# cloudflare/sliceslice-rs

Hardware: AMD Instinct MI355X
Metric: haystack GB/s scanned (and % HBM roofline), 16-byte needle, 1/2/4/8 MI355X (higher is better)
Workload: dtype u8

## Files before the change

sliceslice-rs_amd/csrc/batched_kernels.hpp:

```cpp
#pragma once
#include "batched_types.hpp"

namespace ss {

constexpr uint32_t kPlanSliceMajorMax = 8;

constexpr uint32_t kPlanSampleTiles = 1024, kPlanSampleBytes = 4096, kPlanSampleBlocks = 64;
__device__ __forceinline__ uint8_t class_from_count(uint32_t cnt, uint32_t total)
{
    if (cnt == 0) return 0;
    const uint32_t ratio = total / cnt;
    const uint32_t bits = 31u - (uint32_t)__builtin_clz(ratio);
    return (uint8_t)(15u - (bits < 15u ? bits : 15u));
}
struct BatchClasses {
    uint32_t hist[256];
    uint32_t done, pad[15];
    uint8_t cls[256];
};
__global__ void __launch_bounds__(kBlock) batch_sample_kernel(const uint8_t *haystacks, const uint64_t *hay_begin, const uint64_t *hay_end,
                                                               uint64_t count, BatchClasses *out, unsigned long long *h_tag,
                                                               unsigned long long tag)
{
    __shared__ uint32_t h[kWavesPerBlock][256];
    __shared__ uint32_t s_total;
    __shared__ int s_last;
    for (int k = threadIdx.x; k < kWavesPerBlock * 256; k += kBlock) (&h[0][0])[k] = 0;
    if (threadIdx.x == 0) s_total = 0;
    __syncthreads();
    const int lane = threadIdx.x & (kWave - 1), wave = threadIdx.x / kWave;
    constexpr uint32_t kPerWave = kPlanSampleTiles / (kPlanSampleBlocks * kWavesPerBlock);
    for (uint32_t t = 0; t < kPerWave; ++t) {
        const uint64_t j = ((uint64_t)blockIdx.x * kWavesPerBlock + wave) * kPerWave + t;
        if (count < kPlanSampleTiles && j >= count * ((kPlanSampleTiles + count - 1) / count)) break;
        const uint64_t prob = count >= kPlanSampleTiles ? j * count / kPlanSampleTiles : j % count;
        const uint64_t h0 = hay_begin[prob], h1 = hay_end[prob];
        if (h1 <= h0) continue;
        const uint64_t len = h1 - h0;
        uint64_t off = 0, take = len;
        if (len > kPlanSampleBytes) {
            const uint64_t frac = ((uint32_t)j * 2654435761u) >> 8;
            off = (uint64_t)(((unsigned __int128)(len - kPlanSampleBytes) * frac) >> 24);
            take = kPlanSampleBytes;
        } else if (count < kPlanSampleTiles && j >= count) {
            continue;
        }
        const uint8_t *p = haystacks + h0 + off + (uint64_t)lane * 64;
        const uint64_t mine = (uint64_t)lane * 64 < take ? take - (uint64_t)lane * 64 : 0;
        if (mine >= 64) {
#pragma unroll
            for (int q = 0; q < 16; ++q) {
                const uint32_t w = reinterpret_cast<const UnalignedU32 *>(p + 4 * q)->v;
                atomicAdd(&h[wave][w & 0xFF], 1u);
                atomicAdd(&h[wave][(w >> 8) & 0xFF], 1u);
                atomicAdd(&h[wave][(w >> 16) & 0xFF], 1u);
                atomicAdd(&h[wave][w >> 24], 1u);
            }
        } else {
            for (uint64_t q = 0; q < mine; ++q) atomicAdd(&h[wave][p[q]], 1u);
        }
    }
    __syncthreads();
    const uint32_t part = h[0][threadIdx.x] + h[1][threadIdx.x] + h[2][threadIdx.x] + h[3][threadIdx.x];
    if (part) __hip_atomic_fetch_add(&out->hist[threadIdx.x], part, __ATOMIC_RELAXED, __HIP_MEMORY_SCOPE_AGENT);
    __threadfence();
    __syncthreads();
    if (threadIdx.x == 0)
        s_last = __hip_atomic_fetch_add(&out->done, 1u, __ATOMIC_ACQ_REL, __HIP_MEMORY_SCOPE_AGENT) + 1u == kPlanSampleBlocks;
    __syncthreads();
    if (!s_last) return;
    __threadfence();
    const uint32_t mine = __hip_atomic_exchange(&out->hist[threadIdx.x], 0u, __ATOMIC_RELAXED, __HIP_MEMORY_SCOPE_AGENT);
    uint32_t sum = mine;
#pragma unroll
    for (int o = 32; o > 0; o >>= 1) sum += __shfl_xor(sum, o);
    if (lane == 0) atomicAdd(&s_total, sum);
    __syncthreads();
    out->cls[threadIdx.x] = class_from_count(mine, s_total);
    __threadfence_system();
    __syncthreads();
    if (threadIdx.x == 0) {
        __hip_atomic_store(&out->done, 0u, __ATOMIC_RELAXED, __HIP_MEMORY_SCOPE_AGENT);
        if (h_tag) __hip_atomic_store(h_tag, tag, __ATOMIC_RELEASE, __HIP_MEMORY_SCOPE_SYSTEM);
    }
}

__global__ void __launch_bounds__(kBlock) batch_plan_kernel(const BatchArgs a, uint64_t count, BatchDesc *descs,
                                                             uint32_t nslices, uint32_t min_tiles, int tile_pieces, PlanStats *stats,
                                                             const uint8_t *cls, BatchCold *colds)
{
    __shared__ uint8_t s_class[256];
    __shared__ uint32_t s_max, s_maxt;
    __shared__ unsigned long long s_sum;
    if (threadIdx.x == 0) {
        s_max = s_maxt = 0;
        s_sum = 0;
    }
    if (cls) {
        s_class[threadIdx.x] = cls[threadIdx.x];
    } else {
        constexpr ClassPlanes P = make_class_planes();
        const uint32_t t = threadIdx.x, w = t >> 5;
        uint32_t lo = P.lo[0], hi = P.hi[0];
#pragma unroll
        for (uint32_t k = 1; k < 8; ++k) {
            lo = w == k ? P.lo[k] : lo;
            hi = w == k ? P.hi[k] : hi;
        }
        s_class[t] = (uint8_t)(((lo >> (t & 31)) & 1u) | (((hi >> (t & 31)) & 1u) << 1));
    }
    const uint64_t prob = (uint64_t)blockIdx.x * kBlock + threadIdx.x;
    const bool live = prob < count;
    const uint64_t pi = live ? prob : 0;
    const uint64_t h0 = a.hay_begin[pi], h1 = a.hay_end[pi];
    const uint64_t n0 = a.needle_begin[pi], n1 = a.needle_end[pi];
    const uint64_t given = a.position ? a.position[pi] : 0;
    __syncthreads();
    uint64_t tiles = 0;
    const bool free_pair = cls != nullptr && a.position == nullptr;
    if (stats) {
        uint32_t eff = 0;
        if (live) eff = plan_one(a, pi, h0, h1, n0, n1, given, descs, nslices, min_tiles, tile_pieces, s_class, &tiles, free_pair, colds);
        if (eff != 0) {
            atomicMax(&s_max, eff);
            atomicMax(&s_maxt, tiles > 0xffffffffull ? 0xffffffffu : (uint32_t)tiles);
            atomicAdd(&s_sum, (unsigned long long)tiles);
        }
        __syncthreads();
        if (threadIdx.x == 0 && s_max != 0) {
            atomicMax(&stats->max_slices, s_max);
            atomicMax(&stats->max_tiles, s_maxt);
            atomicAdd(reinterpret_cast<unsigned long long *>(&stats->total_tiles), s_sum);
        }
        return;
    }
    if (live) (void)plan_one(a, pi, h0, h1, n0, n1, given, descs, nslices, min_tiles, tile_pieces, s_class, &tiles, free_pair, colds);
}

__global__ void __launch_bounds__(kBlock) batch_cold_kernel(const BatchArgs a, const BatchDesc *__restrict__ descs, uint64_t count,
                                                             BatchCold *colds, const uint8_t *cls, int find)
{
    __shared__ uint8_t s_class[256];
    if (cls) {
        s_class[threadIdx.x] = cls[threadIdx.x];
    } else {
        s_class[threadIdx.x] = (uint8_t)rarity_class4((uint8_t)threadIdx.x);
    }
    __syncthreads();
    const uint64_t prob = (uint64_t)blockIdx.x * kBlock + threadIdx.x;
    if (prob >= count) return;
    const BatchDesc d = descs[prob];
    BatchCold c;
    c.order_idx[0] = c.order_idx[1] = c.order_val[0] = c.order_val[1] = 0;
    c.tail16[0] = c.tail16[1] = c.tail16[2] = c.tail16[3] = 0;
    c.norder = c.exact_len = 0;
    c.pad[0] = c.pad[1] = find ? ~0u : 0u;
    if ((d.per >> 32) != 0 && ((d.bytes >> 24) & 1) == 0) {
        const uint8_t *needle = a.needles + d.needle_off + d.anchor;
        const uint64_t nrel = d.n - d.anchor;
        const uint32_t lim = nrel < (uint64_t)kRefineWindow ? (uint32_t)nrel : (uint32_t)kRefineWindow;
        const uint32_t pos2 = 4 * ((d.shifts >> 6) & 3) + ((d.shifts >> 4) & 3), pos3 = 4 * ((d.shifts >> 10) & 3) + ((d.shifts >> 8) & 3);
        uint32_t b[kRefineWindow], k[kRefineWindow];
#pragma unroll
        for (int K = 0; K < kRefineWindow; ++K) b[K] = needle[(uint32_t)K < lim ? K : 0];
#pragma unroll
        for (int K = 0; K < kRefineWindow; ++K) k[K] = s_class[b[K]];
        uint32_t valid = 0;
#pragma unroll
        for (int K = 1; K < kRefineWindow; ++K)
            if ((uint32_t)K < lim && (uint32_t)K != pos2 && (uint32_t)K != pos3) valid |= 1u << K;
        uint64_t i0 = 0, i1 = 0, v0 = 0, v1 = 0;
        uint32_t m = 0, used = 0, far_used = 0;
        auto emit = [&](uint32_t K, uint32_t byte) {
            const uint32_t sh = 8 * (m & 7);
            if (m < 8) { i0 |= (uint64_t)K << sh; v0 |= (uint64_t)byte << sh; }
            else { i1 |= (uint64_t)K << sh; v1 |= (uint64_t)byte << sh; }
            ++m;
            used |= 1u << K;
        };
#pragma unroll 1
        for (uint32_t cl = 0; cl < 16; ++cl) {
#pragma unroll
            for (int K = 16; K < kRefineWindow; ++K)
                if (((valid >> K) & 1u) && k[K] == cl && far_used < kFarFirst) { emit(K, b[K]); ++far_used; }
        }
#pragma unroll 1
        for (uint32_t cl = 0; cl < 16; ++cl) {
#pragma unroll
            for (int K = 1; K < 16; ++K)
                if (((valid >> K) & 1u) && k[K] == cl && m < 15) emit(K, b[K]);
        }
#pragma unroll 1
        for (uint32_t cl = 0; cl < 16; ++cl) {
#pragma unroll
            for (int K = 16; K < kRefineWindow; ++K)
                if (((valid >> K) & 1u) && !((used >> K) & 1u) && k[K] == cl && m < 15) emit(K, b[K]);
        }
        c.norder = m;
        c.order_idx[0] = i0; c.order_idx[1] = i1;
        c.order_val[0] = v0; c.order_val[1] = v1;
        if (nrel <= 16) {
            const uint32_t behind = (uint32_t)nrel;
            const uint32_t back = (uint32_t)(d.anchor < 16 - behind ? d.anchor : 16 - behind);
            const uint32_t el = behind + back;
            c.exact_len = el | (back << 8);
            uint32_t t[16];
#pragma unroll
            for (uint32_t j = 0; j < 16; ++j) t[j] = (needle - back)[j < el ? j : 0];
#pragma unroll
            for (uint32_t j = 0; j < 16; ++j) t[j] = j < el ? t[j] : 0u;
#pragma unroll
            for (int j = 0; j < 4; ++j) c.tail16[j] = t[4 * j] | (t[4 * j + 1] << 8) | (t[4 * j + 2] << 16) | (t[4 * j + 3] << 24);
        }
    }
    colds[prob] = c;
}

struct __attribute__((aligned(64))) PlanCtl {
    unsigned long long run_word;
    uint32_t tally[2];
    uint32_t pad[12];
};
static_assert(sizeof(PlanCtl) == 64, "a line of its own");
struct __attribute__((aligned(128))) PlanState {
    struct __attribute__((aligned(64))) Half {
        uint64_t word;
        uint64_t pad[7];
    } half[2];
};
static_assert(sizeof(PlanState) == 128, "a problem's state: a cache line of its own, one half per run parity");
extern "C" __device__ unsigned long long ss_llvm_dispatch_id(void) __asm("llvm.amdgcn.dispatch.id");
__device__ __forceinline__ unsigned long long plan_run_identity()
{
    const uint64_t queue = (uint64_t)(uintptr_t)__builtin_amdgcn_queue_ptr() >> 12;
    return ((queue & 0x7FFFFFFull) << 36) | (ss_llvm_dispatch_id() & ((1ull << 36) - 1ull));
}

#ifndef SS_BATCH_WAVES_MAX
#define SS_BATCH_WAVES_MAX 4
#endif
template <int U, bool FIND = false, bool PLAN = false, bool MULTI = PLAN>
__global__ void __attribute__((amdgpu_waves_per_eu(4, SS_BATCH_WAVES_MAX))) __launch_bounds__(kBlock)
scan_batched_plan_kernel(const BatchArgs a, const BatchDesc *__restrict__ descs, uint32_t count, uint32_t nslices, BatchCold *colds,
                         PlanCtl *ctl, PlanState *states, unsigned long long *h_tally, uint32_t run)
{
    constexpr bool COUNTED = PLAN;
    __shared__ __attribute__((aligned(16))) uint8_t s_needle[kWavesPerBlock * kNeedleLds];
    __shared__ unsigned long long s_wg[kWavesPerBlock];
    const uint32_t w = blockIdx.x;
    const bool slice_major = nslices <= kPlanSliceMajorMax;
    uint32_t prob, slice;
    if (slice_major) {
        slice = w / count;
        prob = w - slice * count;
    } else {
        prob = w / nslices;
        slice = w - prob * nslices;
    }
    BatchCold *rec = colds + prob;
    const BatchDesc *dp = descs + prob;
    const bool peek = !FIND && slice_major && slice != 0;
    int seen0 = 0, seen1 = 0;
    if (MULTI) {
        if (peek) {
            seen0 = __hip_atomic_load(reinterpret_cast<int *>(&states[prob].half[0].word), __ATOMIC_RELAXED, __HIP_MEMORY_SCOPE_AGENT);
            seen1 = __hip_atomic_load(reinterpret_cast<int *>(&states[prob].half[1].word), __ATOMIC_RELAXED, __HIP_MEMORY_SCOPE_AGENT);
        }
    } else if (peek) {
        seen0 = __hip_atomic_load(reinterpret_cast<int *>(&rec->pad[1]), __ATOMIC_RELAXED, __HIP_MEMORY_SCOPE_AGENT);
    }
    BatchDesc d = *dp;
    unsigned long long run_word = 0;
    static_assert(PLAN || !MULTI, "only plans have runs");
    constexpr bool multi = MULTI;
    if (multi) __asm__ volatile("s_load_dwordx2 %0, %1, 0x0\n\ts_waitcnt lgkmcnt(0)" : "=s"(run_word) : "s"(ctl) : "memory");
    if (COUNTED) {
        pin_hot_fields(d);
        if ((threadIdx.x & (kWave - 1)) == 0)
            __hip_atomic_store(&s_wg[threadIdx.x / kWave], FIND ? ~0ull : 0ull, __ATOMIC_RELAXED, __HIP_MEMORY_SCOPE_WORKGROUP);
    }
    uint32_t parity = 0;
    if (multi) {
        const unsigned long long me = plan_run_identity();
        const bool mine = (run_word >> 1) == me;
        parity = mine ? (uint32_t)(run_word & 1ull) : (uint32_t)(run_word & 1ull) ^ 1u;
        if (blockIdx.x == 0 && threadIdx.x == 0 && !mine) {
            if (h_tally) {
                const uint32_t total = __hip_atomic_exchange(&ctl->tally[parity ^ 1u], 0u, __ATOMIC_RELAXED, __HIP_MEMORY_SCOPE_AGENT);
                __hip_atomic_store(h_tally, ((unsigned long long)run << 32) | total, __ATOMIC_RELAXED, __HIP_MEMORY_SCOPE_SYSTEM);
            }
            __hip_atomic_store(&ctl->run_word, (me << 1) | parity, __ATOMIC_RELAXED, __HIP_MEMORY_SCOPE_AGENT);
        }
    }
    const uint32_t eff = (uint32_t)(d.per >> 32), per = (uint32_t)d.per;
    const bool shared = MULTI && eff > 1;
    const int seen = MULTI ? (parity ? seen1 : seen0) : seen0;
    int *found = FIND ? nullptr : (shared ? reinterpret_cast<int *>(&states[prob].half[parity].word) : reinterpret_cast<int *>(&rec->pad[1]));
    void *sink = FIND ? (shared ? static_cast<void *>(&states[prob].half[parity].word) : static_cast<void *>(&rec->pad[0])) : static_cast<void *>(found);
    const uint32_t mis = d.shifts & 15;
    const uint64_t npieces = ((mis + d.end + 15) / 16 + 63) / 64;
    const uint64_t ntiles = (npieces + kWavesPerBlock * U - 1) / (kWavesPerBlock * U);
    if (slice >= eff) {
        if (COUNTED && eff == 0 && slice == 0 && threadIdx.x == 0) {
            if (FIND) a.best[prob] = d.n == 0 ? 0ull : ~0ull;
            else a.found[prob] = (int)d.shifts;
        }
        return;
    }
    uint64_t t0, te, step;
    bool work = true;
    if (slice_major) {
        t0 = (uint64_t)slice * per;
        te = t0 + per < ntiles ? t0 + per : ntiles;
        step = 1;
        work = __builtin_amdgcn_readfirstlane(seen) == 0;
    } else {
        t0 = slice;
        te = ntiles;
        step = eff;
    }
    work = work && t0 < te;
    if (!work) return;
    const bool opener = MULTI && eff > 1 && slice == 0 && threadIdx.x == 0;
    if (opener) {
        __hip_atomic_store(&states[prob].half[parity ^ 1u].word, FIND ? ~0ull : 0ull, __ATOMIC_RELAXED, __HIP_MEMORY_SCOPE_AGENT);
        if (FIND) (void)__hip_atomic_exchange(a.best + prob, ~0ull, __ATOMIC_RELAXED, __HIP_MEMORY_SCOPE_AGENT);
        else (void)__hip_atomic_exchange(a.found + prob, 0, __ATOMIC_RELAXED, __HIP_MEMORY_SCOPE_AGENT);
    }

    if (work) {
        Problem pr;
        hot_problem(d, mis, npieces, pr);
        constexpr bool READY = PLAN;
        typename std::conditional<READY, ColdInPlanT<MULTI>, ColdInCall>::type cold;
        if constexpr (READY)
            cold = ColdInPlanT<MULTI>{dp, colds + prob, a.needles, MULTI && eff > 1 ? (FIND ? static_cast<void *>(a.best + prob) : static_cast<void *>(a.found + prob)) : nullptr,
                              MULTI && eff > 1 && h_tally ? &ctl->tally[parity] : nullptr};
        else cold = ColdInCall{dp, colds + prob, a.needles, FIND ? static_cast<void *>(a.best + prob) : static_cast<void *>(a.found + prob)};
        void *wg_sink = COUNTED && eff == 1 ? static_cast<void *>(&s_wg[threadIdx.x / kWave]) : nullptr;
        if ((d.bytes >> 24) & 1) scan_tiles<0, 0, true, U, 1, FIND, false, true>(pr, cold, s_needle, t0, step, te, sink, wg_sink);
        else scan_tiles<kQDynamic, 0, false, U, 1, FIND, false, true>(pr, cold, s_needle, t0, step, te, sink, wg_sink);
    }
    if (opener) {
        __asm__ volatile("s_waitcnt vmcnt(0)" ::: "memory");
        if (FIND) {
            const uint64_t v = __hip_atomic_load(&states[prob].half[parity].word, __ATOMIC_RELAXED, __HIP_MEMORY_SCOPE_AGENT);
            if (v != ~0ull) __hip_atomic_fetch_min(a.best + prob, v, __ATOMIC_RELAXED, __HIP_MEMORY_SCOPE_AGENT);
        } else {
            const int v = __hip_atomic_load(reinterpret_cast<int *>(&states[prob].half[parity].word), __ATOMIC_RELAXED, __HIP_MEMORY_SCOPE_AGENT);
            if (v != 0) (void)__hip_atomic_exchange(a.found + prob, 1, __ATOMIC_RELAXED, __HIP_MEMORY_SCOPE_AGENT);
        }
    }
    if (COUNTED && eff == 1) {
        __syncthreads();
        if (threadIdx.x == 0) {
            unsigned long long mine = FIND ? ~0ull : 0ull;
#pragma unroll
            for (int k = 0; k < kWavesPerBlock; ++k) {
                const unsigned long long v = __hip_atomic_load(&s_wg[k], __ATOMIC_RELAXED, __HIP_MEMORY_SCOPE_WORKGROUP);
                mine = FIND ? (v < mine ? v : mine) : (mine | v);
            }
            if (FIND) a.best[prob] = mine;
            else a.found[prob] = mine != 0;
            if (MULTI) {
                __hip_atomic_store(&states[prob].half[0].word, FIND ? ~0ull : 0ull, __ATOMIC_RELAXED, __HIP_MEMORY_SCOPE_AGENT);
                __hip_atomic_store(&states[prob].half[1].word, FIND ? ~0ull : 0ull, __ATOMIC_RELAXED, __HIP_MEMORY_SCOPE_AGENT);
            }
        }
    }
}

__global__ void __launch_bounds__(kBlock) scan_pairs_kernel(const BatchArgs a, uint64_t count)
{
    const uint64_t prob = (uint64_t)blockIdx.x * kBlock + threadIdx.x;
    if (prob >= count) return;
    const uint64_t h0 = a.hay_begin[prob], n0 = a.needle_begin[prob];
    const uint64_t len = a.hay_end[prob] - h0, n = a.needle_end[prob] - n0;
    int result = 0;
    uint64_t position = (a.position && n) ? a.position[prob] : n - 1;
    if (n == 0) {
        result = 1;
    } else if (n == 1 ? position != 0 : position >= n) {
        result = kBadPosition;
    } else if (len >= n) {
        const uint8_t *h = a.haystacks + h0, *nd = a.needles + n0;
        const uint8_t first = nd[0], last = nd[position];
        const uint64_t end = len - n + 1;
        for (uint64_t i = 0; i < end && !result; ++i) {
            if (h[i] != first || h[i + position] != last) continue;
            uint64_t k = 1;
            while (k < n && h[i + k] == nd[k]) ++k;
            result = k >= n;
        }
    }
    a.found[prob] = result;
}

}
```

Measured before the change: 7448.

## Load short pair haystacks into registers and search with SWAR word ops

For small problems (haystack up to 32 bytes), scan_pairs_kernel now loads the haystack and needle as aligned 16-byte vector loads into registers. It realigns them with alignbyte and runs a wave-uniform SWAR first/last-byte filter plus a masked word compare. This replaces per-byte global loads and divergent loops. Longer inputs keep the original byte loop, gated by a ballot, at the cost of more register use and extra code for the fallback.

```diff
diff --git a/sliceslice-rs_amd/csrc/batched_kernels.hpp b/sliceslice-rs_amd/csrc/batched_kernels.hpp
--- a/sliceslice-rs_amd/csrc/batched_kernels.hpp
+++ b/sliceslice-rs_amd/csrc/batched_kernels.hpp
@@ -1,5 +1,6 @@
 #pragma once
 #include "batched_types.hpp"
+#include "pairs_word.hpp"
 
 namespace ss {
 
@@ -370,27 +371,45 @@
     }
 }
 
+template <int... K>
+__device__ __forceinline__ void pairs_load_word(const uint8_t *p, uint32_t len, bool take, uint32_t (&raw)[kPairsRaw], std::integer_sequence<int, K...>)
+{
+    const uint32_t s = (uint32_t)(uintptr_t)p & 15u;
+    const uint4 *c = reinterpret_cast<const uint4 *>(p - s);
+    const uint4 v[sizeof...(K)] = {(take && s + len > 16u * K ? c[K] : make_uint4(0, 0, 0, 0))...};
+    ((raw[4 * K] = v[K].x, raw[4 * K + 1] = v[K].y, raw[4 * K + 2] = v[K].z, raw[4 * K + 3] = v[K].w), ...);
+}
+
 __global__ void __launch_bounds__(kBlock) scan_pairs_kernel(const BatchArgs a, uint64_t count)
 {
     const uint64_t prob = (uint64_t)blockIdx.x * kBlock + threadIdx.x;
     if (prob >= count) return;
     const uint64_t h0 = a.hay_begin[prob], n0 = a.needle_begin[prob];
     const uint64_t len = a.hay_end[prob] - h0, n = a.needle_end[prob] - n0;
-    int result = 0;
-    uint64_t position = (a.position && n) ? a.position[prob] : n - 1;
-    if (n == 0) {
-        result = 1;
-    } else if (n == 1 ? position != 0 : position >= n) {
-        result = kBadPosition;
-    } else if (len >= n) {
-        const uint8_t *h = a.haystacks + h0, *nd = a.needles + n0;
-        const uint8_t first = nd[0], last = nd[position];
-        const uint64_t end = len - n + 1;
-        for (uint64_t i = 0; i < end && !result; ++i) {
-            if (h[i] != first || h[i + position] != last) continue;
-            uint64_t k = 1;
-            while (k < n && h[i + k] == nd[k]) ++k;
-            result = k >= n;
+    const uint64_t position = a.position ? a.position[prob] : n - 1;
+    const uint8_t *h = a.haystacks + h0, *nd = a.needles + n0;
+    const bool bad = n != 0 && (n == 1 ? position != 0 : position >= n);
+    const bool search = n != 0 && !bad && len >= n;
+    const bool in_regs = search && len <= (uint64_t)kPairsCap;
+    uint32_t hraw[kPairsRaw], nraw[kPairsRaw];
+    pairs_load_word(h, (uint32_t)len, in_regs, hraw, std::make_integer_sequence<int, kPairsRaw / 4>());
+    pairs_load_word(nd, (uint32_t)n, in_regs, nraw, std::make_integer_sequence<int, kPairsRaw / 4>());
+    uint32_t hw[kPairsDwords], nw[kPairsDwords];
+    pairs_word_align(hraw, (uint32_t)(uintptr_t)h & 15u, hw);
+    pairs_word_align(nraw, (uint32_t)(uintptr_t)nd & 15u, nw);
+    int result = pairs_word_search(hw, in_regs ? (uint32_t)len : 0u, nw, in_regs ? (uint32_t)n : 1u);
+    if (n == 0) result = 1;
+    else if (bad) result = kBadPosition;
+    if (__builtin_amdgcn_ballot_w64(search && !in_regs) != 0) {
+        if (search && !in_regs) {
+            const uint8_t first = nd[0], last = nd[position];
+            const uint64_t end = len - n + 1;
+            for (uint64_t i = 0; i < end && !result; ++i) {
+                if (h[i] != first || h[i + position] != last) continue;
+                uint64_t k = 1;
+                while (k < n && h[i + k] == nd[k]) ++k;
+                result = k >= n;
+            }
         }
     }
     a.found[prob] = result;
diff --git a/sliceslice-rs_amd/csrc/pairs_word.hpp b/sliceslice-rs_amd/csrc/pairs_word.hpp
--- /dev/null
+++ b/sliceslice-rs_amd/csrc/pairs_word.hpp
@@ -0,0 +1,98 @@
+#pragma once
+#include <stdint.h>
+
+#include <utility>
+
+#if defined(__HIPCC__) || defined(__CUDACC__)
+#define SS_PW_HD __host__ __device__ __forceinline__
+#else
+#define SS_PW_HD inline
+#endif
+
+namespace ss {
+
+constexpr int kPairsCap = 32;
+constexpr int kPairsDwords = kPairsCap / 4;
+constexpr int kPairsRaw = kPairsCap / 4 + 4;
+
+SS_PW_HD uint32_t pw_alignbyte(uint32_t hi, uint32_t lo, uint32_t s)
+{
+#if defined(__HIP_DEVICE_COMPILE__)
+    return __builtin_amdgcn_alignbyte(hi, lo, s);
+#else
+    s &= 3u;
+    return s ? (lo >> (8u * s)) | (hi << (32u - 8u * s)) : lo;
+#endif
+}
+
+SS_PW_HD bool pw_any(bool x)
+{
+#if defined(__HIP_DEVICE_COMPILE__)
+    return __builtin_amdgcn_ballot_w64(x) != 0;
+#else
+    return x;
+#endif
+}
+
+SS_PW_HD uint32_t pw_mask(uint32_t n, int k)
+{
+    const int b = (int)n - 4 * k;
+    return b <= 0 ? 0u : b >= 4 ? ~0u : (1u << (8 * b)) - 1u;
+}
+
+template <int D, int N, int... I>
+SS_PW_HD void pw_move_down(const uint32_t (&in)[N + D], bool up, uint32_t (&out)[N], std::integer_sequence<int, I...>)
+{
+    ((out[I] = up ? in[I + D] : in[I]), ...);
+}
+
+SS_PW_HD void pairs_word_align(const uint32_t (&raw)[kPairsRaw], uint32_t s, uint32_t (&out)[kPairsDwords])
+{
+    uint32_t a[kPairsRaw - 2], b[kPairsRaw - 3];
+    pw_move_down<2, kPairsRaw - 2>(raw, (s & 8u) != 0, a, std::make_integer_sequence<int, kPairsRaw - 2>());
+    pw_move_down<1, kPairsRaw - 3>(a, (s & 4u) != 0, b, std::make_integer_sequence<int, kPairsRaw - 3>());
+#pragma unroll
+    for (int i = 0; i < kPairsDwords; ++i) out[i] = pw_alignbyte(b[i + 1], b[i], s);
+}
+
+template <int K>
+SS_PW_HD uint32_t pw_differ(const uint32_t (&w)[kPairsDwords + 1], const uint32_t (&nd)[kPairsDwords], uint32_t n, uint32_t r, bool pass)
+{
+    if constexpr (K >= kPairsDwords) {
+        return 0;
+    } else {
+        if (K > 1 && !pw_any(pass && n > 4u * K)) return 0;
+        const uint32_t wk = r ? pw_alignbyte(w[K + 1], w[K], r) : w[K];
+        return ((wk ^ nd[K]) & pw_mask(n, K)) | pw_differ<K + 1>(w, nd, n, r, pass);
+    }
+}
+
+SS_PW_HD bool pairs_word_search(const uint32_t (&h)[kPairsDwords], uint32_t len, const uint32_t (&nd)[kPairsDwords], uint32_t n)
+{
+    const int last = (int)len - (int)n;
+    const uint32_t m0 = pw_mask(n, 0), n0 = nd[0] & m0;
+    uint32_t w[kPairsDwords + 1];
+#pragma unroll
+    for (int k = 0; k < kPairsDwords; ++k) w[k] = h[k];
+    w[kPairsDwords] = 0;
+    const uint32_t j = n < 4u ? (n ? n - 1u : 0u) : 3u;
+    const uint32_t first = (nd[0] & 0xffu) * 0x01010101u, second = (nd[0] >> (8u * j) & 0xffu) * 0x01010101u;
+    bool found = false;
+    for (int g = 0; g < kPairsDwords && pw_any(!found && 4 * g <= last); ++g) {
+        const uint32_t x = (w[0] ^ first) | (pw_alignbyte(w[1], w[0], j) ^ second);
+        const uint32_t z = n ? (x - 0x01010101u) & ~x & 0x80808080u : 0x80808080u;
+#pragma unroll
+        for (int r = 0; r < 4; ++r) {
+            if (!pw_any((z >> (8 * r + 7) & 1u) != 0 && 4 * g + r <= last)) continue;
+            const uint32_t w0 = r ? pw_alignbyte(w[1], w[0], (uint32_t)r) : w[0];
+            bool pass = (w0 & m0) == n0 && 4 * g + r <= last;
+            if (pw_any(pass && n > 4)) pass = pass && pw_differ<1>(w, nd, n, (uint32_t)r, pass) == 0;
+            found = found || pass;
+        }
+#pragma unroll
+        for (int k = 0; k < kPairsDwords; ++k) w[k] = w[k + 1];
+    }
+    return found;
+}
+
+}
```

After: 7447 (median of 2 runs). Within noise of the previous version (-0.0%).
